# anerisheth19/CNN-MobileNet-V1-implementation-on-AWS-FPGA-using-OpenCL

Hardware: AMD Instinct MI355X
Metric: images/sec MobileNet-V1 1.0x224 fp32, batch 256; per-stage HBM GB/s vs roofline (higher is better)
Workload: dtype f32

## Files before the change

### cnn-mobilenet-v1-implementation-on-aws-fpga-using-opencl_amd/csrc/mbn_f32_stem.hip

```cpp
#include "mbn_internal.h"
#include "mbn_epilogue.h"
#include "mbn_x6.h"

namespace {

constexpr int TH = MBN_STEM_TH, TW = MBN_STEM_TW;
constexpr int CR = TH + 2, CC = TW + 2;
constexpr int PR = 2 * CR + 1;
constexpr int PROW = 112;
constexpr int PROWPAD = 4;

struct StemArgs {

    float *out;
    const float *in, *w1, *s1, *b1, *wd, *s2, *b2, *wp, *s3, *b3;
    const uint8_t *in8;
    int batch, rows, cols;
    int oh, ow;
    int tiles_y, tiles_x;
    unsigned ntiles;
};

template <int C1>
__device__ __forceinline__ int swz(int row, int chunk)
{
    if (C1 == 32) return (row << 5) + (((chunk ^ (row >> 1)) & 7) << 2);
    return (row << 4) + (((chunk ^ (row >> 2)) & 3) << 2);
}
template <int C1>
__device__ __forceinline__ int swzb(int row, int slot)
{
    if (C1 == 32) return (row << 4) + (((slot ^ (row >> 2)) & 3) << 2);
    return (row << 3) + (((slot ^ (row >> 3)) & 1) << 2);
}
__device__ __forceinline__ f4 fma4(float x, f4 w, f4 acc) { return __builtin_elementwise_fma(f4{ x, x, x, x }, w, acc); }
__device__ __forceinline__ f4 fma4v(f4 x, f4 w, f4 acc) { return __builtin_elementwise_fma(x, w, acc); }

constexpr int PAIRS = PROW / 2;
constexpr int NPF = (PR * PAIRS + 255) / 256;

__device__ __forceinline__ void patch_load(const StemArgs &a, unsigned t, int tid, f2 (&pf)[NPF])
{
    const int tx = (int)(t % (unsigned)a.tiles_x);
    const unsigned q0 = t / (unsigned)a.tiles_x;
    const int ty = (int)(q0 % (unsigned)a.tiles_y);
    const long n = q0 / (unsigned)a.tiles_y;
    const long img = n * a.rows * a.cols * 3;
    const int iy0 = 2 * (TH * ty - 1), fx0 = 6 * (TW * tx - 1), rowf = a.cols * 3;
    const unsigned img_elems = (unsigned)(a.rows * a.cols * 3);
    if (a.in8) {
        const __amdgpu_buffer_rsrc_t rsrc = mbn_make_rsrc(a.in8 + img, img_elems);
#pragma unroll
        for (int k = 0; k < NPF; k++) {
            const int i = tid + k * 256, r = i / PAIRS, j = i % PAIRS;
            const int iy = iy0 + r, fx = fx0 + 2 * j;
            const bool ok = i < PR * PAIRS && iy >= 0 && iy < a.rows && fx >= 0 && fx < rowf;
            const unsigned u = (unsigned short)__builtin_amdgcn_raw_buffer_load_b16(rsrc, ok ? (unsigned)(iy * rowf + fx) : MBN_OOB, 0, 0);
            pf[k] = ok ? f2{ fmaf((float)(u & 0xff), 1.0f / 127.5f, -1.0f), fmaf((float)(u >> 8), 1.0f / 127.5f, -1.0f) } : f2{ 0.f, 0.f };
        }
    } else {
        const __amdgpu_buffer_rsrc_t rsrc = mbn_make_rsrc(a.in + img, img_elems * 4u);
#pragma unroll
        for (int k = 0; k < NPF; k++) {
            const int i = tid + k * 256, r = i / PAIRS, j = i % PAIRS;
            const int iy = iy0 + r, fx = fx0 + 2 * j;
            const bool ok = i < PR * PAIRS && iy >= 0 && iy < a.rows && fx >= 0 && fx < rowf;
            pf[k] = __builtin_bit_cast(f2, __builtin_amdgcn_raw_buffer_load_b64(rsrc, ok ? (unsigned)(iy * rowf + fx) * 4u : MBN_OOB, 0, 0));
        }
    }
}
__device__ __forceinline__ void patch_store(float *in_s, int tid, const f2 (&pf)[NPF])
{
#pragma unroll
    for (int k = 0; k < NPF; k++) {
        const int i = tid + k * 256;
        if (i < PR * PAIRS) *reinterpret_cast<f2 *>(in_s + 2 * i) = pf[k];
    }
}

__device__ __forceinline__ float rbf(float v) { return (float)(__bf16)v; }
__device__ __forceinline__ f4 rbf4(f4 v) { return f4{ rbf(v.x), rbf(v.y), rbf(v.z), rbf(v.w) }; }
template <int C1, int C3, bool BF, int WPE, bool MC = false, int X6 = 0, bool PADC = true>
__global__ __launch_bounds__(256, WPE) void stem_fused_f32(StemArgs a)
{
    static_assert(!MC || BF || C1 == 32, "conv1 on the MFMA: bf16 mode (16x16x32 bf16, split operands), or fp32 alpha = 1 (16x16x4 fp32)");
    constexpr bool MCF = MC && !BF;
    static_assert(X6 == 0 || (!BF && (X6 == 6 || X6 == 9)), "split products: fp32 mode, 6 or 9 of them");
    constexpr int APL = TH * TW * C1 / 2, BPL = C3 * C1 / 2;
    constexpr int MH = C1 / 16;
    constexpr bool WDL = WPE >= 3;
    constexpr int Q1 = C1 / 4;
    constexpr int PB = 3 * Q1 / 4;
    static_assert(CC % PB == 0 && CR * (CC / PB) * Q1 <= 256, "conv1 lane mapping");
    constexpr int NXV = (3 * (2 * PB + 1) + 3) / 4;
    constexpr int PC = 128 * Q1 / 256;
    constexpr int NI = C3 / 32;
    constexpr int KG = C1 / 8;
    constexpr bool BREG = !BF && X6 == 0 && WPE >= 3 && C1 == 32;
    __shared__ __attribute__((aligned(16))) float in_s[PR * PROW + PROWPAD];
    __shared__ __attribute__((aligned(16))) float w1_s[27 * C1];
    constexpr int C1P = (MCF && C1 == 32 && PADC) ? 40 : C1;
    __shared__ __attribute__((aligned(16))) float c1_s[CR * CC * C1P];
    __shared__ __attribute__((aligned(16))) float a_s[X6 ? 3 * APL : TH * TW * C1 / (BF ? 2 : 1)];
    __shared__ __attribute__((aligned(16))) float b_s[BREG ? 4 : X6 ? 3 * BPL : C3 * C1 / (BF ? 2 : 1)];
    __shared__ __attribute__((aligned(16))) float sb_s[4 * C1];
    __shared__ __attribute__((aligned(16))) float wd_s[WDL ? 9 * C1 : 4];

    const int tid = threadIdx.x, lane = tid & 63, wave = tid >> 6, li = lane & 31, lh = lane >> 5;
    const int c4 = tid % Q1;

    for (int i = tid * 4; i < 27 * C1; i += 1024) *reinterpret_cast<f4 *>(w1_s + i) = *reinterpret_cast<const f4 *>(a.w1 + i);
    if (BF) {
        constexpr int SL = C1 / 8;
        if (tid < C3 * SL) {
            const int row = tid / SL, slot = tid % SL, ch = NI == 2 ? 2 * (row & 31) + (row >> 5) : row;
            *reinterpret_cast<f4 *>(b_s + swzb<C1>(row, slot)) =
                *reinterpret_cast<const f4 *>(reinterpret_cast<const __bf16 *>(a.wp) + ch * C1 + slot * 8);
        }
    } else if constexpr (X6 != 0) {
        constexpr int SL = C1 / 8;
        if (tid < C3 * SL) {
            const int row = tid / SL, slot = tid % SL;
            const float *src = a.wp + row * C1 + slot * 8;
            u4 hw, mw, lw;
            mbn_x6_split8(*reinterpret_cast<const f4 *>(src), *reinterpret_cast<const f4 *>(src + 4), hw, mw, lw);
            *reinterpret_cast<u4 *>(b_s + swzb<C1>(row, slot)) = hw;
            *reinterpret_cast<u4 *>(b_s + BPL + swzb<C1>(row, slot)) = mw;
            *reinterpret_cast<u4 *>(b_s + 2 * BPL + swzb<C1>(row, slot)) = lw;
        }
    } else if constexpr (!BREG)
    for (int i = tid; i < C3 * Q1; i += 256) {
        const int row = i / Q1, ch = i % Q1;
        *reinterpret_cast<f4 *>(b_s + swz<C1>(row, ch)) = *reinterpret_cast<const f4 *>(a.wp + row * C1 + ch * 4);
    }
    [[maybe_unused]] f4 bfr[BREG ? KG : 1][NI];
    if constexpr (BREG) {
#pragma unroll
        for (int g = 0; g < KG; g++)
#pragma unroll
            for (int ni = 0; ni < NI; ni++) bfr[g][ni] = *reinterpret_cast<const f4 *>(a.wp + (ni * 32 + (tid & 31)) * C1 + (2 * g + ((tid & 63) >> 5)) * 4);
    }
    if (tid < 4 * C1) {
        const float *src = tid < C1 ? a.s1 : tid < 2 * C1 ? a.b1 : tid < 3 * C1 ? a.s2 : a.b2;
        sb_s[tid] = src[tid & (C1 - 1)];
    }
    f4 wd[WDL ? 1 : 9];
    if constexpr (WDL) {
        for (int i = tid * 4; i < 9 * C1; i += 1024) *reinterpret_cast<f4 *>(wd_s + i) = *reinterpret_cast<const f4 *>(a.wd + i);
    } else {
#pragma unroll
        for (int k = 0; k < 9; k++) wd[k] = *reinterpret_cast<const f4 *>(a.wd + k * C1 + c4 * 4);
    }
    float s3[NI], b3[NI];
#pragma unroll
    for (int ni = 0; ni < NI; ni++) {
        const int ch = (BF && NI == 2) ? 2 * li + ni : ni * 32 + li;
        s3[ni] = a.s3[ch]; b3[ni] = a.b3[ch];
    }

    f2 pf[NPF];
    if (blockIdx.x < a.ntiles) {
        patch_load(a, blockIdx.x, tid, pf);
        patch_store(in_s, tid, pf);
    }
    __syncthreads();

    [[maybe_unused]] int mc_dl[8];
    [[maybe_unused]] unsigned mc_kok = 0;
    [[maybe_unused]] bf8 mc_wh[MH], mc_wl[MH];
    [[maybe_unused]] f4 mc_s1[MH], mc_b1[MH];
    [[maybe_unused]] int mcf_dl[7];
    [[maybe_unused]] float mcf_w[2][7];
    [[maybe_unused]] f4 mcf_s1[2], mcf_b1[2];
    if constexpr (MCF) {
        const int kg = lane >> 4, pc = lane & 15;
#pragma unroll
        for (int t = 0; t < 7; t++) {
            const int k = 4 * t + kg;
            mcf_dl[t] = k < 27 ? (k / 9) * PROW + (k % 9) : 0;
#pragma unroll
            for (int h = 0; h < 2; h++) mcf_w[h][t] = k < 27 ? w1_s[k * C1 + 16 * h + pc] : 0.f;
        }
#pragma unroll
        for (int h = 0; h < 2; h++) {
            mcf_s1[h] = *reinterpret_cast<const f4 *>(sb_s + 16 * h + 4 * kg);
            mcf_b1[h] = *reinterpret_cast<const f4 *>(sb_s + C1 + 16 * h + 4 * kg);
        }
    }
    if constexpr (MC && BF) {
        const int kg = lane >> 4, pc = lane & 15;
        unsigned whb[MH][8], wlb[MH][8];
#pragma unroll
        for (int j = 0; j < 8; j++) {
            const int k = 8 * kg + j;
            mc_dl[j] = (k / 9) * PROW + (k % 9);
            if (k < 27) mc_kok |= 1u << j;
#pragma unroll
            for (int h = 0; h < MH; h++) {
                const float w = k < 27 ? w1_s[k * C1 + 16 * h + pc] : 0.f;
                const unsigned wb = __builtin_bit_cast(unsigned, w) & 0xffff0000u;
                whb[h][j] = wb;
                wlb[h][j] = __builtin_bit_cast(unsigned, w - __builtin_bit_cast(float, wb));
            }
        }
#pragma unroll
        for (int h = 0; h < MH; h++) {
            u4 ph, pl;
#pragma unroll
            for (int i = 0; i < 4; i++) {
                ph[i] = (whb[h][2 * i] >> 16) | (whb[h][2 * i + 1] & 0xffff0000u);
                pl[i] = (wlb[h][2 * i] >> 16) | (wlb[h][2 * i + 1] & 0xffff0000u);
            }
            mc_wh[h] = __builtin_bit_cast(bf8, ph);
            mc_wl[h] = __builtin_bit_cast(bf8, pl);
            mc_s1[h] = *reinterpret_cast<const f4 *>(sb_s + 16 * h + 4 * kg);
            mc_b1[h] = *reinterpret_cast<const f4 *>(sb_s + C1 + 16 * h + 4 * kg);
        }
    }

    const int bpg = tid / Q1, br = bpg / (CC / PB), bc = (bpg % (CC / PB)) * PB;
    const int cy = (tid / Q1) / (TW / PC), cx = ((tid / Q1) % (TW / PC)) * PC;

    for (unsigned t = blockIdx.x; t < a.ntiles; t += gridDim.x) {
        const int tx = (int)(t % (unsigned)a.tiles_x);
        const unsigned q0 = t / (unsigned)a.tiles_x;
        const int ty = (int)(q0 % (unsigned)a.tiles_y);
        const long n = q0 / (unsigned)a.tiles_y;
        const unsigned tnext = t + gridDim.x;
        if (tnext < a.ntiles) patch_load(a, tnext, tid, pf);

        __builtin_amdgcn_s_setprio(2);
        if constexpr (MCF) {
            const int kg = lane >> 4, pc = lane & 15;
#pragma unroll 1
            for (int bi = 0; bi < 3; bi++) {
                const int blk = wave * 3 + bi;
                const int q = 16 * blk + pc, p = min(q, CR * CC - 1);
                const int r = (p * 3641) >> 16, c = p - r * CC;
                const float *src = in_s + (2 * r) * PROW + 6 * c;
                float xv[7];
#pragma unroll
                for (int t = 0; t < 7; t++) xv[t] = src[mcf_dl[t]];
                if (kg == 3) xv[6] = 0.f;
                const int oy = TH * ty - 1 + r, ox = TW * tx - 1 + c;
                const bool inside = oy >= 0 && oy < a.oh && ox >= 0 && ox < a.ow;
#pragma unroll
                for (int h = 0; h < 2; h++) {
                    f4 acc = f4{ 0.f, 0.f, 0.f, 0.f };
#pragma unroll
                    for (int t = 0; t < 7; t++) acc = __builtin_amdgcn_mfma_f32_16x16x4f32(mcf_w[h][t], xv[t], acc, 0, 0, 0);
                    const f4 v = inside ? mbn_bn_relu6(acc, mcf_s1[h], mcf_b1[h]) : f4{ 0.f, 0.f, 0.f, 0.f };
                    if (q < CR * CC) *reinterpret_cast<f4 *>(c1_s + q * C1P + 16 * h + 4 * kg) = v;
                }
            }
        } else
        if constexpr (MC) {
            const int kg = lane >> 4, pc = lane & 15;
#pragma unroll 1
            for (int bi = 0; bi < 3; bi++) {
                const int blk = wave * 3 + bi;
                const int q = 16 * blk + pc, p = min(q, CR * CC - 1);
                const int r = (p * 3641) >> 16, c = p - r * CC;
                const float *src = in_s + (2 * r) * PROW + 6 * c;
                unsigned xb[8], lb[8];
#pragma unroll
                for (int j = 0; j < 8; j++) {
                    const float x = ((mc_kok >> j) & 1u) ? src[mc_dl[j]] : 0.f;
                    xb[j] = __builtin_bit_cast(unsigned, x) & 0xffff0000u;
                    lb[j] = __builtin_bit_cast(unsigned, x - __builtin_bit_cast(float, xb[j]));
                }
                u4 ph, pl;
#pragma unroll
                for (int i = 0; i < 4; i++) {
                    ph[i] = (xb[2 * i] >> 16) | (xb[2 * i + 1] & 0xffff0000u);
                    pl[i] = (lb[2 * i] >> 16) | (lb[2 * i + 1] & 0xffff0000u);
                }
                const bf8 xh = __builtin_bit_cast(bf8, ph), xl = __builtin_bit_cast(bf8, pl);
                const int oy = TH * ty - 1 + r, ox = TW * tx - 1 + c;
                const bool inside = oy >= 0 && oy < a.oh && ox >= 0 && ox < a.ow;
#pragma unroll
                for (int h = 0; h < MH; h++) {
                    f4 acc = f4{ 0.f, 0.f, 0.f, 0.f };
                    acc = __builtin_amdgcn_mfma_f32_16x16x32_bf16(mc_wl[h], xh, acc, 0, 0, 0);
                    acc = __builtin_amdgcn_mfma_f32_16x16x32_bf16(mc_wh[h], xl, acc, 0, 0, 0);
                    acc = __builtin_amdgcn_mfma_f32_16x16x32_bf16(mc_wh[h], xh, acc, 0, 0, 0);
                    const f4 v = inside ? rbf4(mbn_bn_relu6(acc, mc_s1[h], mc_b1[h])) : f4{ 0.f, 0.f, 0.f, 0.f };
                    if (q < CR * CC) *reinterpret_cast<f4 *>(c1_s + q * C1 + 16 * h + 4 * kg) = v;
                }
            }
        } else
        if (bpg < CR * (CC / PB)) {
            f4 acc[PB];
#pragma unroll
            for (int p = 0; p < PB; p++) acc[p] = f4{ 0.f, 0.f, 0.f, 0.f };
#pragma unroll 1
            for (int ky = 0; ky < 3; ky++) {
                const float *row = in_s + (2 * br + ky) * PROW + (2 * bc) * 3;
                float x[4 * NXV];
                if constexpr (PB == 6) {
#pragma unroll
                    for (int j = 0; j < NXV; j++) {
                        const f4 t = *reinterpret_cast<const f4 *>(row + 4 * j);
                        x[4 * j] = t.x; x[4 * j + 1] = t.y; x[4 * j + 2] = t.z; x[4 * j + 3] = t.w;
                    }
                } else {
#pragma unroll
                    for (int j = 0; j < 2 * NXV - 1; j++) {
                        const f2 t = *reinterpret_cast<const f2 *>(row + 2 * j);
                        x[2 * j] = t.x; x[2 * j + 1] = t.y;
                    }
                }
#pragma unroll
                for (int kx = 0; kx < 3; kx++)
#pragma unroll
                    for (int ci = 0; ci < 3; ci++) {
                        const f4 w = *reinterpret_cast<const f4 *>(w1_s + ((ky * 3 + kx) * 3 + ci) * C1 + c4 * 4);
#pragma unroll
                        for (int p = 0; p < PB; p++) acc[p] = fma4(x[(2 * p + kx) * 3 + ci], w, acc[p]);
                    }
            }
            const int oy = TH * ty - 1 + br, ox = TW * tx - 1 + bc;
            const bool rowok = oy >= 0 && oy < a.oh;
            const f4 s1 = *reinterpret_cast<const f4 *>(sb_s + c4 * 4), b1 = *reinterpret_cast<const f4 *>(sb_s + C1 + c4 * 4);
#pragma unroll
            for (int p = 0; p < PB; p++) {
                f4 v = (rowok && ox + p >= 0 && ox + p < a.ow) ? mbn_bn_relu6(acc[p], s1, b1) : f4{ 0.f, 0.f, 0.f, 0.f };
                if (BF) v = rbf4(v);
                *reinterpret_cast<f4 *>(c1_s + (br * CC + bc + p) * C1 + c4 * 4) = v;
            }
        }
        __syncthreads();
        if (tnext < a.ntiles) patch_store(in_s, tid, pf);

        {
            f4 acc[PC];
#pragma unroll
            for (int p = 0; p < PC; p++) acc[p] = f4{ 0.f, 0.f, 0.f, 0.f };
#pragma unroll
            for (int dy = 0; dy < 3; dy++) {
                f4 v[PC + 2];
#pragma unroll
                for (int j = 0; j < PC + 2; j++) v[j] = *reinterpret_cast<const f4 *>(c1_s + ((cy + dy) * CC + cx + j) * C1P + c4 * 4);
#pragma unroll
                for (int dx = 0; dx < 3; dx++) {
                    f4 wt;
                    if constexpr (WDL) wt = *reinterpret_cast<const f4 *>(wd_s + (dy * 3 + dx) * C1 + c4 * 4);
                    else wt = wd[dy * 3 + dx];
#pragma unroll
                    for (int p = 0; p < PC; p++) acc[p] = fma4v(v[p + dx], wt, acc[p]);
                }
            }
            const f4 s2 = *reinterpret_cast<const f4 *>(sb_s + 2 * C1 + c4 * 4), b2 = *reinterpret_cast<const f4 *>(sb_s + 3 * C1 + c4 * 4);
#pragma unroll
            for (int p = 0; p < PC; p++) {
                const f4 v = mbn_bn_relu6(acc[p], s2, b2);
                if (BF) {
                    const int row = cy * TW + cx + p;
                    *reinterpret_cast<bf4 *>(a_s + swzb<C1>(row, c4 >> 1) + 2 * (c4 & 1)) = bf4{ (__bf16)v.x, (__bf16)v.y, (__bf16)v.z, (__bf16)v.w };
                } else if constexpr (X6 != 0) {
                    const int o = swzb<C1>(cy * TW + cx + p, c4 >> 1) + 2 * (c4 & 1);
                    u2 hw, mw, lw;
                    mbn_x6_split4(v, hw, mw, lw);
                    *reinterpret_cast<u2 *>(a_s + o) = hw;
                    *reinterpret_cast<u2 *>(a_s + APL + o) = mw;
                    *reinterpret_cast<u2 *>(a_s + 2 * APL + o) = lw;
                } else *reinterpret_cast<f4 *>(a_s + swz<C1>(cy * TW + cx + p, c4)) = v;
            }
        }
        __syncthreads();

        __builtin_amdgcn_s_setprio(0);
        f16v acc[NI];
#pragma unroll
        for (int ni = 0; ni < NI; ni++)
#pragma unroll
            for (int r = 0; r < 16; r++) acc[ni][r] = 0.f;
        if constexpr (BF) {
#pragma unroll
            for (int ks = 0; ks < C1 / 16; ks++) {
                const f4 av = *reinterpret_cast<const f4 *>(a_s + swzb<C1>(wave * 32 + li, 2 * ks + lh));
#pragma unroll
                for (int ni = 0; ni < NI; ni++) {
                    const f4 bv = *reinterpret_cast<const f4 *>(b_s + swzb<C1>(ni * 32 + li, 2 * ks + lh));
                    acc[ni] = __builtin_amdgcn_mfma_f32_32x32x16_bf16(__builtin_bit_cast(bf8, av), __builtin_bit_cast(bf8, bv), acc[ni], 0, 0, 0);
                }
            }
            const __amdgpu_buffer_rsrc_t orsrc = mbn_make_rsrc(reinterpret_cast<__bf16 *>(a.out) + n * a.oh * a.ow * C3, (unsigned)(a.oh * a.ow * C3 * 2));
            const unsigned lane_off = (unsigned)(4 * lh * C3) * 2u + (unsigned)li * (NI == 2 ? 4u : 2u);
#pragma unroll
            for (int r = 0; r < 16; r++) {
                const int y = TH * ty + 2 * __builtin_amdgcn_readfirstlane(wave) + (r >> 3), x = TW * tx + (r & 3) + 8 * ((r >> 2) & 1);
                const unsigned soff = (unsigned)((y * a.ow + x) * C3) * 2u;
                if constexpr (NI == 2) {
                    const float v0 = mbn_relu6(fmaf(acc[0][r], s3[0], b3[0])), v1 = mbn_relu6(fmaf(acc[1][r], s3[1], b3[1]));
                    __builtin_amdgcn_raw_buffer_store_b32(__builtin_bit_cast(unsigned, bf2{ (__bf16)v0, (__bf16)v1 }), orsrc, lane_off, soff, 0);
                } else {
                    __builtin_amdgcn_raw_buffer_store_b16(__builtin_bit_cast(unsigned short, (__bf16)mbn_relu6(fmaf(acc[0][r], s3[0], b3[0]))), orsrc, lane_off, soff, 0);
                }
            }
        } else {
        if constexpr (X6 != 0) {
            constexpr int pa9[9] = { 2, 2, 1, 2, 0, 1, 1, 0, 0 }, pb9[9] = { 2, 1, 2, 0, 2, 1, 0, 1, 0 };
            constexpr int pa6[6] = { 2, 0, 1, 1, 0, 0 }, pb6[6] = { 0, 2, 1, 0, 1, 0 };
#pragma unroll
            for (int ks = 0; ks < C1 / 16; ks++) {
                f4 av[3], bv[3][NI];
#pragma unroll
                for (int pl = 0; pl < 3; pl++) {
                    av[pl] = *reinterpret_cast<const f4 *>(a_s + pl * APL + swzb<C1>(wave * 32 + li, 2 * ks + lh));
#pragma unroll
                    for (int ni = 0; ni < NI; ni++) bv[pl][ni] = *reinterpret_cast<const f4 *>(b_s + pl * BPL + swzb<C1>(ni * 32 + li, 2 * ks + lh));
                }
#pragma unroll
                for (int q = 0; q < X6; q++)
#pragma unroll
                    for (int ni = 0; ni < NI; ni++)
                        acc[ni] = __builtin_amdgcn_mfma_f32_32x32x16_bf16(__builtin_bit_cast(bf8, av[X6 == 6 ? pa6[q % 6] : pa9[q]]),
                                                                          __builtin_bit_cast(bf8, bv[X6 == 6 ? pb6[q % 6] : pb9[q]][ni]), acc[ni], 0, 0, 0);
            }
        } else
#pragma unroll
        for (int g = 0; g < KG; g++) {
            const int chunk = 2 * g + lh;
            const f4 av = *reinterpret_cast<const f4 *>(a_s + swz<C1>(wave * 32 + li, chunk));
            f4 bv[NI];
#pragma unroll
            for (int ni = 0; ni < NI; ni++) {
                if constexpr (BREG) bv[ni] = bfr[g][ni];
                else bv[ni] = *reinterpret_cast<const f4 *>(b_s + swz<C1>(ni * 32 + li, chunk));
            }
#pragma unroll
            for (int s = 0; s < 4; s++)
#pragma unroll
                for (int ni = 0; ni < NI; ni++) acc[ni] = __builtin_amdgcn_mfma_f32_32x32x2f32(av[s], bv[ni][s], acc[ni], 0, 0, 0);
        }
        if constexpr (C1 == 32 && !BREG) {
            float *obase = a.out + ((n * a.oh + TH * ty) * a.ow + TW * tx) * C3;
#pragma unroll
            for (int ni = 0; ni < NI; ni++)
#pragma unroll
                for (int r = 0; r < 16; r++) {
                    const int q = wave * 32 + (r & 3) + 8 * (r >> 2) + 4 * lh;
                    const int y = q >> 4, x = q & 15;
                    obase[((long)y * a.ow + x) * C3 + ni * 32 + li] = mbn_relu6(fmaf(acc[ni][r], s3[ni], b3[ni]));
                }
        } else {
        const __amdgpu_buffer_rsrc_t orsrc = mbn_make_rsrc(a.out + n * a.oh * a.ow * C3, (unsigned)(a.oh * a.ow * C3 * 4));
        const unsigned lane_off = (unsigned)(4 * lh * C3 + li) * 4u;
#pragma unroll
        for (int ni = 0; ni < NI; ni++)
#pragma unroll
            for (int r = 0; r < 16; r++) {
                const int y = TH * ty + 2 * __builtin_amdgcn_readfirstlane(wave) + (r >> 3), x = TW * tx + (r & 3) + 8 * ((r >> 2) & 1);
                const unsigned soff = (unsigned)((y * a.ow + x) * C3 + ni * 32) * 4u;
                __builtin_amdgcn_raw_buffer_store_b32(__builtin_bit_cast(unsigned, mbn_relu6(fmaf(acc[ni][r], s3[ni], b3[ni]))), orsrc, lane_off, soff, 0);
            }
        }
        }
    }
}

}

int mbn_launch_f32_stem(mbn_context *ctx, hipStream_t stream, float *out, const float *in, const float *w1,
                        const float *s1, const float *b1, const float *wd, const float *s2, const float *b2,
                        const float *wp, const float *s3, const float *b3, int batch, int rows, int cols, int c1, int c3, int in_u8, int bf16)
{
    StemArgs a;
    a.in8 = in_u8 ? (const uint8_t *)in : nullptr;
    a.out = out; a.in = in; a.w1 = w1; a.s1 = s1; a.b1 = b1; a.wd = wd; a.s2 = s2; a.b2 = b2; a.wp = wp; a.s3 = s3; a.b3 = b3;
    a.batch = batch; a.rows = rows; a.cols = cols; a.oh = rows / 2; a.ow = cols / 2;
    a.tiles_y = a.oh / TH; a.tiles_x = a.ow / TW;
    a.ntiles = (unsigned)((long)batch * a.tiles_y * a.tiles_x);
    const int wpe_bf = g_mbn_tune.misc == 2 ? 2 : 3;
    const int per_cu = c1 == 16 ? 4 : (bf16 ? wpe_bf : 2);
    long grid = (long)ctx->num_cus * per_cu;
    if (grid > (long)a.ntiles) grid = (long)a.ntiles;
    const dim3 g((unsigned)grid), b(256);
    if (c1 == 32) {
#ifdef MBN_LAB
        if (bf16 && wpe_bf == 3 && g_mbn_tune.conv_variant == 2) hipLaunchKernelGGL((stem_fused_f32<32, 64, true, 3>), g, b, 0, stream, a);
        else if (bf16 && wpe_bf != 3) hipLaunchKernelGGL((stem_fused_f32<32, 64, true, 2>), g, b, 0, stream, a);
        else
#endif
        if (bf16) hipLaunchKernelGGL((stem_fused_f32<32, 64, true, 3, true>), g, b, 0, stream, a);
        else if (g_mbn_tune.pw_emul == 6) hipLaunchKernelGGL((stem_fused_f32<32, 64, false, 2, true, 6>), g, b, 0, stream, a);
        else if (g_mbn_tune.pw_emul == 9) hipLaunchKernelGGL((stem_fused_f32<32, 64, false, 2, true, 9>), g, b, 0, stream, a);
#ifdef MBN_LAB
        else if (g_mbn_tune.conv_variant == 3 || g_mbn_tune.conv_variant == 4) {
            long g3 = (long)ctx->num_cus * (g_mbn_tune.conv_variant == 3 ? 3 : 2);
            if (g3 > (long)a.ntiles) g3 = (long)a.ntiles;
            hipLaunchKernelGGL((stem_fused_f32<32, 64, false, 3>), dim3((unsigned)g3), b, 0, stream, a);
        }
#endif
#ifdef MBN_LAB
        else if (g_mbn_tune.conv_variant == 6) hipLaunchKernelGGL((stem_fused_f32<32, 64, false, 2, true, 0, false>), g, b, 0, stream, a);
        else if (g_mbn_tune.conv_variant == 5) hipLaunchKernelGGL((stem_fused_f32<32, 64, false, 2>), g, b, 0, stream, a);
#endif
        else hipLaunchKernelGGL((stem_fused_f32<32, 64, false, 2, true>), g, b, 0, stream, a);
    } else {
#ifdef MBN_LAB
        if (bf16 && g_mbn_tune.conv_variant == 2) hipLaunchKernelGGL((stem_fused_f32<16, 32, true, 4>), g, b, 0, stream, a);
        else
#endif
        if (bf16) {
            long g5 = (long)ctx->num_cus * 5;
            if (g5 > (long)a.ntiles) g5 = (long)a.ntiles;
            hipLaunchKernelGGL((stem_fused_f32<16, 32, true, 5, true>), dim3((unsigned)g5), b, 0, stream, a);
        }
        else if (g_mbn_tune.pw_emul == 6) hipLaunchKernelGGL((stem_fused_f32<16, 32, false, 4, false, 6>), g, b, 0, stream, a);
        else if (g_mbn_tune.pw_emul == 9) hipLaunchKernelGGL((stem_fused_f32<16, 32, false, 4, false, 9>), g, b, 0, stream, a);
        else hipLaunchKernelGGL((stem_fused_f32<16, 32, false, 4>), g, b, 0, stream, a);
    }
    return MBN_OK;
}
```

Measured before the change: 91660.

## Software-pipeline stem conv1 across tiles with a u8 input path in MFMA fp32 mode

For the fp32 MFMA conv1 stem variant, the kernel is restructured so that the next tile's conv1 and its global patch load run during the current tile's tail, in a two-tile-deep prefetch. Tile index math is hoisted into a helper, and the shared buffers are padded so the branch-free conv1 writes need no bounds guard. A templated uint8 input path loads 16-bit pairs and normalizes them in registers, with dedicated launches when the input is u8. The output store is rewritten with per-wave row pointers and immediate offsets. This adds register and LDS pressure and a more complex schedule, in exchange for overlapping input latency and conv1 compute with the pointwise stage.

```diff
diff --git a/cnn-mobilenet-v1-implementation-on-aws-fpga-using-opencl_amd/csrc/mbn_f32_stem.hip b/cnn-mobilenet-v1-implementation-on-aws-fpga-using-opencl_amd/csrc/mbn_f32_stem.hip
--- a/cnn-mobilenet-v1-implementation-on-aws-fpga-using-opencl_amd/csrc/mbn_f32_stem.hip
+++ b/cnn-mobilenet-v1-implementation-on-aws-fpga-using-opencl_amd/csrc/mbn_f32_stem.hip
@@ -78,9 +78,62 @@
     }
 }
 
+constexpr int PFS = 256 * NPF;
+constexpr int C1DUMP = 16 * 12 - CR * CC;
+struct StemTile { int ty, tx; long n; };
+__device__ __forceinline__ StemTile stem_tile(const StemArgs &a, unsigned t)
+{
+    const unsigned q0 = t / (unsigned)a.tiles_x;
+    return StemTile{ (int)(q0 % (unsigned)a.tiles_y), (int)(t % (unsigned)a.tiles_x), (long)(q0 / (unsigned)a.tiles_y) };
+}
+struct StemPatch { f2 f[NPF]; unsigned short u[NPF]; unsigned ok; };
+template <bool U8>
+__device__ __forceinline__ void patch_load_sl(const StemArgs &a, const StemTile &tl, int tid, StemPatch &pf)
+{
+    const long img = tl.n * a.rows * a.cols * 3;
+    const int iy0 = 2 * (TH * tl.ty - 1), fx0 = 6 * (TW * tl.tx - 1), rowf = a.cols * 3;
+    const unsigned img_elems = (unsigned)(a.rows * a.cols * 3);
+    if constexpr (U8) {
+        pf.ok = 0;
+        const __amdgpu_buffer_rsrc_t rsrc = mbn_make_rsrc(a.in8 + img, img_elems);
+#pragma unroll
+        for (int k = 0; k < NPF; k++) {
+            const int i = tid + k * 256, r = i / PAIRS, j = i % PAIRS;
+            const int iy = iy0 + r, fx = fx0 + 2 * j;
+            const bool ok = (i < PR * PAIRS) & ((unsigned)iy < (unsigned)a.rows) & ((unsigned)fx < (unsigned)rowf);
+            pf.u[k] = (unsigned short)__builtin_amdgcn_raw_buffer_load_b16(rsrc, ok ? (unsigned)(iy * rowf + fx) : MBN_OOB, 0, 0);
+            pf.ok |= ok ? 1u << k : 0u;
+        }
+    } else {
+        const __amdgpu_buffer_rsrc_t rsrc = mbn_make_rsrc(a.in + img, img_elems * 4u);
+#pragma unroll
+        for (int k = 0; k < NPF; k++) {
+            const int i = tid + k * 256, r = i / PAIRS, j = i % PAIRS;
+            const int iy = iy0 + r, fx = fx0 + 2 * j;
+            const bool ok = (i < PR * PAIRS) & ((unsigned)iy < (unsigned)a.rows) & ((unsigned)fx < (unsigned)rowf);
+            pf.f[k] = __builtin_bit_cast(f2, __builtin_amdgcn_raw_buffer_load_b64(rsrc, ok ? (unsigned)(iy * rowf + fx) * 4u : MBN_OOB, 0, 0));
+        }
+    }
+}
+template <bool U8>
+__device__ __forceinline__ void patch_store_sl(float *in_s, int tid, const StemPatch &pf)
+{
+    if constexpr (U8) {
+#pragma unroll
+        for (int k = 0; k < NPF; k++) {
+            const unsigned u = pf.u[k];
+            const f2 v = f2{ fmaf((float)(u & 0xff), 1.0f / 127.5f, -1.0f), fmaf((float)(u >> 8), 1.0f / 127.5f, -1.0f) };
+            *reinterpret_cast<f2 *>(in_s + 2 * (tid + k * 256)) = ((pf.ok >> k) & 1u) ? v : f2{ 0.f, 0.f };
+        }
+    } else {
+#pragma unroll
+        for (int k = 0; k < NPF; k++) *reinterpret_cast<f2 *>(in_s + 2 * (tid + k * 256)) = pf.f[k];
+    }
+}
+
 __device__ __forceinline__ float rbf(float v) { return (float)(__bf16)v; }
 __device__ __forceinline__ f4 rbf4(f4 v) { return f4{ rbf(v.x), rbf(v.y), rbf(v.z), rbf(v.w) }; }
-template <int C1, int C3, bool BF, int WPE, bool MC = false, int X6 = 0, bool PADC = true>
+template <int C1, int C3, bool BF, int WPE, bool MC = false, int X6 = 0, bool PADC = true, bool U8 = false>
 __global__ __launch_bounds__(256, WPE) void stem_fused_f32(StemArgs a)
 {
     static_assert(!MC || BF || C1 == 32, "conv1 on the MFMA: bf16 mode (16x16x32 bf16, split operands), or fp32 alpha = 1 (16x16x4 fp32)");
@@ -97,10 +150,13 @@
     constexpr int NI = C3 / 32;
     constexpr int KG = C1 / 8;
     constexpr bool BREG = !BF && X6 == 0 && WPE >= 3 && C1 == 32;
-    __shared__ __attribute__((aligned(16))) float in_s[PR * PROW + PROWPAD];
+    constexpr bool SL = MCF;
+    static_assert(SL || !U8, "only the SL forms take the input type as a template parameter");
+    static_assert(2 * PFS >= PR * PROW + PROWPAD, "the padded patch covers the plain one");
+    __shared__ __attribute__((aligned(16))) float in_s[SL ? 2 * PFS : PR * PROW + PROWPAD];
     __shared__ __attribute__((aligned(16))) float w1_s[27 * C1];
     constexpr int C1P = (MCF && C1 == 32 && PADC) ? 40 : C1;
-    __shared__ __attribute__((aligned(16))) float c1_s[CR * CC * C1P];
+    __shared__ __attribute__((aligned(16))) float c1_s[(CR * CC + (SL ? C1DUMP : 0)) * C1P];
     __shared__ __attribute__((aligned(16))) float a_s[X6 ? 3 * APL : TH * TW * C1 / (BF ? 2 : 1)];
     __shared__ __attribute__((aligned(16))) float b_s[BREG ? 4 : X6 ? 3 * BPL : C3 * C1 / (BF ? 2 : 1)];
     __shared__ __attribute__((aligned(16))) float sb_s[4 * C1];
@@ -158,8 +214,15 @@
         s3[ni] = a.s3[ch]; b3[ni] = a.b3[ch];
     }
 
-    f2 pf[NPF];
-    if (blockIdx.x < a.ntiles) {
+    [[maybe_unused]] f2 pf[NPF];
+    [[maybe_unused]] StemTile tcur{}, tnx{};
+    [[maybe_unused]] StemPatch sp;
+    if constexpr (SL) {
+        if (blockIdx.x >= a.ntiles) return;
+        tcur = stem_tile(a, blockIdx.x);
+        patch_load_sl<U8>(a, tcur, tid, sp);
+        patch_store_sl<U8>(in_s, tid, sp);
+    } else if (blockIdx.x < a.ntiles) {
         patch_load(a, blockIdx.x, tid, pf);
         patch_store(in_s, tid, pf);
     }
@@ -221,39 +284,52 @@
     const int bpg = tid / Q1, br = bpg / (CC / PB), bc = (bpg % (CC / PB)) * PB;
     const int cy = (tid / Q1) / (TW / PC), cx = ((tid / Q1) % (TW / PC)) * PC;
 
+    [[maybe_unused]] auto conv1_mcf = [&](int ty, int tx) {
+        const int kg = lane >> 4, pc = lane & 15;
+#pragma unroll 1
+        for (int bi = 0; bi < 3; bi++) {
+            const int blk = wave * 3 + bi;
+            const int q = 16 * blk + pc, p = min(q, CR * CC - 1);
+            const int r = (p * 3641) >> 16, c = p - r * CC;
+            const float *src = in_s + (2 * r) * PROW + 6 * c;
+            float xv[7];
+#pragma unroll
+            for (int t = 0; t < 7; t++) xv[t] = src[mcf_dl[t]];
+            xv[6] = kg == 3 ? 0.f : xv[6];
+            const int oy = TH * ty - 1 + r, ox = TW * tx - 1 + c;
+            const bool inside = ((unsigned)oy < (unsigned)a.oh) & ((unsigned)ox < (unsigned)a.ow);
+#pragma unroll
+            for (int h = 0; h < 2; h++) {
+                f4 acc = f4{ 0.f, 0.f, 0.f, 0.f };
+#pragma unroll
+                for (int t = 0; t < 7; t++) acc = __builtin_amdgcn_mfma_f32_16x16x4f32(mcf_w[h][t], xv[t], acc, 0, 0, 0);
+                const f4 bn = mbn_bn_relu6(acc, mcf_s1[h], mcf_b1[h]);
+                *reinterpret_cast<f4 *>(c1_s + q * C1P + 16 * h + 4 * kg) = inside ? bn : f4{ 0.f, 0.f, 0.f, 0.f };
+            }
+        }
+    };
+    if constexpr (SL) {
+        const unsigned t1 = blockIdx.x + gridDim.x;
+        tnx = stem_tile(a, t1 < a.ntiles ? t1 : blockIdx.x);
+        patch_load_sl<U8>(a, tnx, tid, sp);
+        conv1_mcf(tcur.ty, tcur.tx);
+        __builtin_amdgcn_s_waitcnt(0x0f70);
+    }
+
     for (unsigned t = blockIdx.x; t < a.ntiles; t += gridDim.x) {
-        const int tx = (int)(t % (unsigned)a.tiles_x);
+        int tx, ty;
+        long n;
+        [[maybe_unused]] unsigned tnext = 0;
+        if constexpr (SL) { tx = tcur.tx; ty = tcur.ty; n = tcur.n; }
+        else {
+        tx = (int)(t % (unsigned)a.tiles_x);
         const unsigned q0 = t / (unsigned)a.tiles_x;
-        const int ty = (int)(q0 % (unsigned)a.tiles_y);
-        const long n = q0 / (unsigned)a.tiles_y;
-        const unsigned tnext = t + gridDim.x;
+        ty = (int)(q0 % (unsigned)a.tiles_y);
+        n = q0 / (unsigned)a.tiles_y;
+        tnext = t + gridDim.x;
         if (tnext < a.ntiles) patch_load(a, tnext, tid, pf);
 
         __builtin_amdgcn_s_setprio(2);
-        if constexpr (MCF) {
-            const int kg = lane >> 4, pc = lane & 15;
-#pragma unroll 1
-            for (int bi = 0; bi < 3; bi++) {
-                const int blk = wave * 3 + bi;
-                const int q = 16 * blk + pc, p = min(q, CR * CC - 1);
-                const int r = (p * 3641) >> 16, c = p - r * CC;
-                const float *src = in_s + (2 * r) * PROW + 6 * c;
-                float xv[7];
-#pragma unroll
-                for (int t = 0; t < 7; t++) xv[t] = src[mcf_dl[t]];
-                if (kg == 3) xv[6] = 0.f;
-                const int oy = TH * ty - 1 + r, ox = TW * tx - 1 + c;
-                const bool inside = oy >= 0 && oy < a.oh && ox >= 0 && ox < a.ow;
-#pragma unroll
-                for (int h = 0; h < 2; h++) {
-                    f4 acc = f4{ 0.f, 0.f, 0.f, 0.f };
-#pragma unroll
-                    for (int t = 0; t < 7; t++) acc = __builtin_amdgcn_mfma_f32_16x16x4f32(mcf_w[h][t], xv[t], acc, 0, 0, 0);
-                    const f4 v = inside ? mbn_bn_relu6(acc, mcf_s1[h], mcf_b1[h]) : f4{ 0.f, 0.f, 0.f, 0.f };
-                    if (q < CR * CC) *reinterpret_cast<f4 *>(c1_s + q * C1P + 16 * h + 4 * kg) = v;
-                }
-            }
-        } else
         if constexpr (MC) {
             const int kg = lane >> 4, pc = lane & 15;
 #pragma unroll 1
@@ -329,8 +405,12 @@
                 *reinterpret_cast<f4 *>(c1_s + (br * CC + bc + p) * C1 + c4 * 4) = v;
             }
         }
+        }
         __syncthreads();
-        if (tnext < a.ntiles) patch_store(in_s, tid, pf);
+        if constexpr (SL) {
+            patch_store_sl<U8>(in_s, tid, sp);
+            __builtin_amdgcn_s_setprio(2);
+        } else if (tnext < a.ntiles) patch_store(in_s, tid, pf);
 
         {
             f4 acc[PC];
@@ -434,15 +514,24 @@
 #pragma unroll
                 for (int ni = 0; ni < NI; ni++) acc[ni] = __builtin_amdgcn_mfma_f32_32x32x2f32(av[s], bv[ni][s], acc[ni], 0, 0, 0);
         }
+        if constexpr (SL) {
+            const unsigned t1 = t + gridDim.x, t2 = t1 < a.ntiles ? t1 + gridDim.x : t;
+            const StemTile tnn = stem_tile(a, t2 < a.ntiles ? t2 : t);
+            patch_load_sl<U8>(a, tnn, tid, sp);
+            conv1_mcf(tnx.ty, tnx.tx);
+            tcur = tnx; tnx = tnn;
+        }
         if constexpr (C1 == 32 && !BREG) {
-            float *obase = a.out + ((n * a.oh + TH * ty) * a.ow + TW * tx) * C3;
+            const int ws = __builtin_amdgcn_readfirstlane(wave);
+            char *row0 = reinterpret_cast<char *>(a.out + ((n * a.oh + TH * ty + 2 * ws) * a.ow + TW * tx) * C3);
+            char *row1 = row0 + (long)a.ow * (C3 * 4);
+            const unsigned lane_off = (unsigned)(4 * lh * C3 + li) * 4u;
 #pragma unroll
             for (int ni = 0; ni < NI; ni++)
 #pragma unroll
                 for (int r = 0; r < 16; r++) {
-                    const int q = wave * 32 + (r & 3) + 8 * (r >> 2) + 4 * lh;
-                    const int y = q >> 4, x = q & 15;
-                    obase[((long)y * a.ow + x) * C3 + ni * 32 + li] = mbn_relu6(fmaf(acc[ni][r], s3[ni], b3[ni]));
+                    const int imm = (((r & 3) + 8 * ((r >> 2) & 1)) * C3 + ni * 32) * 4;
+                    *reinterpret_cast<float *>(((r >> 3) ? row1 : row0) + (size_t)lane_off + imm) = mbn_relu6(fmaf(acc[ni][r], s3[ni], b3[ni]));
                 }
         } else {
         const __amdgpu_buffer_rsrc_t orsrc = mbn_make_rsrc(a.out + n * a.oh * a.ow * C3, (unsigned)(a.oh * a.ow * C3 * 4));
@@ -484,8 +573,13 @@
         else
 #endif
         if (bf16) hipLaunchKernelGGL((stem_fused_f32<32, 64, true, 3, true>), g, b, 0, stream, a);
-        else if (g_mbn_tune.pw_emul == 6) hipLaunchKernelGGL((stem_fused_f32<32, 64, false, 2, true, 6>), g, b, 0, stream, a);
-        else if (g_mbn_tune.pw_emul == 9) hipLaunchKernelGGL((stem_fused_f32<32, 64, false, 2, true, 9>), g, b, 0, stream, a);
+        else if (g_mbn_tune.pw_emul == 6) {
+            if (in_u8) hipLaunchKernelGGL((stem_fused_f32<32, 64, false, 2, true, 6, true, true>), g, b, 0, stream, a);
+            else hipLaunchKernelGGL((stem_fused_f32<32, 64, false, 2, true, 6>), g, b, 0, stream, a);
+        } else if (g_mbn_tune.pw_emul == 9) {
+            if (in_u8) hipLaunchKernelGGL((stem_fused_f32<32, 64, false, 2, true, 9, true, true>), g, b, 0, stream, a);
+            else hipLaunchKernelGGL((stem_fused_f32<32, 64, false, 2, true, 9>), g, b, 0, stream, a);
+        }
 #ifdef MBN_LAB
         else if (g_mbn_tune.conv_variant == 3 || g_mbn_tune.conv_variant == 4) {
             long g3 = (long)ctx->num_cus * (g_mbn_tune.conv_variant == 3 ? 3 : 2);
@@ -494,9 +588,10 @@
         }
 #endif
 #ifdef MBN_LAB
-        else if (g_mbn_tune.conv_variant == 6) hipLaunchKernelGGL((stem_fused_f32<32, 64, false, 2, true, 0, false>), g, b, 0, stream, a);
+        else if (g_mbn_tune.conv_variant == 6 && !in_u8) hipLaunchKernelGGL((stem_fused_f32<32, 64, false, 2, true, 0, false>), g, b, 0, stream, a);
         else if (g_mbn_tune.conv_variant == 5) hipLaunchKernelGGL((stem_fused_f32<32, 64, false, 2>), g, b, 0, stream, a);
 #endif
+        else if (in_u8) hipLaunchKernelGGL((stem_fused_f32<32, 64, false, 2, true, 0, true, true>), g, b, 0, stream, a);
         else hipLaunchKernelGGL((stem_fused_f32<32, 64, false, 2, true>), g, b, 0, stream, a);
     } else {
 #ifdef MBN_LAB
```

Result: no change. 91620 (-0.0%).
